# cmgcds/SParSH-AMG

Hardware: NVIDIA B200
Metric: amg_pcg_solve_seconds_poisson3d_256 (lower is better)
Workload: dtype f64

## Files before the change

### sparsh_amg_b200/csrc/internal.cuh

```cuda
#pragma once
#include <cuda_runtime.h>
#include <stdint.h>

#include <string>

#include <nvtx3/nvToolsExt.h>

#include "../../include/sparsh_b200.h"

namespace sparsh {

void set_error(const std::string &msg);
int cuda_fail(cudaError_t e, const char *what, const char *file, int line);

#define SP_CUDA(call)                                                              \
    do {                                                                           \
        cudaError_t e__ = (call);                                                  \
        if (e__ != cudaSuccess) return ::sparsh::cuda_fail(e__, #call, __FILE__, __LINE__); \
    } while (0)
#define SP_TRY(call)                      \
    do {                                  \
        int rc__ = (call);                \
        if (rc__ != SPARSH_OK) return rc__; \
    } while (0)
// ... 82 lines not shown
    int off;
    int pad;
};
struct PatView {
    const unsigned char *__restrict__ pat;
    const PatEntry *__restrict__ ent;
    const int *__restrict__ start;
    const double *__restrict__ pdiag;
    int n_pat, n_ent;
    int use_pdiag;
    int far_off;
};
constexpr int PAT_TILE = 512;
constexpr int PAT_MAX_WIN = 8;
constexpr int PAT_WIN_DOUBLES = 3072;
struct PatWindows {
    int nwin;
    int lo[PAT_MAX_WIN], len[PAT_MAX_WIN];
    int total;
    int w0;
    const unsigned char *__restrict__ win;
};
constexpr int PAT0_MAX = 32;
struct Pat0 {
    int len = 0;
    int kdiag = -1;
    int lo = 0, hi = 0;
    double diag = 0.0;
    double cover = 0.0;
    int off[PAT0_MAX] = {};
    double val[PAT0_MAX] = {};
};
constexpr int PAT_ESCAPE = 255;
constexpr int PAT_MAX_ENT = 2048;
constexpr int PAT_MAX_ROW = 64;

struct CsrView {
    int nrow, ncol, nnz;
    const int *__restrict__ rowptr;
    const int *__restrict__ col;
    const double *__restrict__ val;
};

}

struct sparsh_matrix_s {
    int nrow = 0, ncol = 0, nnz = 0;
    int *rowptr = nullptr;
    int *col = nullptr;
    double *val = nullptr;
    double *diag = nullptr;
    int kind = sparsh::KIND_VECTOR;
    int threads = 256;
    bool threads_forced = false;
    int lanes = 8;
    int max_row = 0;
    double mean_row = 0.0;
    int win128 = 0, win256 = 0;
    int smem_bytes = 0;
    unsigned short *code = nullptr;
    double *dict_val = nullptr;
    int *dict_off = nullptr;
    int n_dval = 0, n_doff = 0;
    bool has_dict = false;
    unsigned char *pat = nullptr;
    sparsh::PatEntry *pat_ent = nullptr;
// ... 113 lines not shown
```

### sparsh_amg_b200/csrc/matrix.cu

```cuda
#include <algorithm>
#include <chrono>
#include <cmath>
#include <cstdlib>
#include <cstring>
#include <mutex>
#include <thread>
#include <unordered_map>
#include <vector>

#include <cstdio>

#include "spmv_common.cuh"

using namespace sparsh;

namespace {

void choose_kernel(sparsh_matrix_s *A, const int *rp) {
    const int n = A->nrow;
    int max_row = 0, w128 = 0, w256 = 0;
    for (int i = 0; i < n; i++) {
        max_row = std::max(max_row, rp[i + 1] - rp[i]);
        w128 = std::max(w128, rp[std::min(i + 128, n)] - rp[i]);
        w256 = std::max(w256, rp[std::min(i + 256, n)] - rp[i]);
// ... 795 lines not shown
    if (smem_bytes) *smem_bytes = A->kind == KIND_STREAM ? A->smem_bytes : 0;
    if (smem_bytes && A->kind == KIND_DICT)
        *smem_bytes = ((((A->threads == 256 ? A->win256 : A->win128) + 16) + 7) & ~7) * 2 + A->n_dval * 8 + A->n_doff * 4;
    return SPARSH_OK;
}

int sparsh_matrix_pattern_stats(sparsh_matrix_t A, int *n_pat, int *n_ent, int *n_escape, double *cover0) {
    SP_REQUIRE(A != nullptr, "matrix is NULL");
    if (n_pat) *n_pat = A->has_pat ? A->n_pat : 0;
    if (n_ent) *n_ent = A->has_pat ? A->n_pent : 0;
    if (n_escape) *n_escape = A->has_pat ? A->n_escape : A->nrow;
    if (cover0) *cover0 = A->has_pat ? A->pat0.cover : 0.0;
    return SPARSH_OK;
}

int sparsh_matrix_kernel_name(sparsh_matrix_t A, int epi, char *buf, size_t len) {
    SP_REQUIRE(A != nullptr && buf != nullptr && len > 0, "bad arguments");
    static const char *epis[] = {"EPI_SPMV", "EPI_RESID", "EPI_JACOBI", "EPI_PROLONG", "EPI_SOR", "EPI_SPMV_DOT", "EPI_RESNORM"};
    SP_REQUIRE(epi >= 0 && epi < 7, "unknown epilogue");
    char tmp[160];
    switch (A->kind) {
        case KIND_SCALAR:
            std::snprintf(tmp, sizeof tmp, "csr_scalar_kernel<256,%s>", epis[epi]);
            break;
        case KIND_STREAM:
            std::snprintf(tmp, sizeof tmp, "csr_stream_kernel<%d,%s>", A->threads, epis[epi]);
            break;
        case KIND_DICT:
            std::snprintf(tmp, sizeof tmp, "csr_dict_kernel<%d,4,%s>", A->threads, epis[epi]);
            break;
        case KIND_PATTERN:
            if (pattern_lean_applies(A)) {
                const bool div = epi == EPI_JACOBI || epi == EPI_SOR;
                const bool one_row = A->threads_forced ? A->threads == 256 : div;
                std::snprintf(tmp, sizeof tmp, "csr_pat2_kernel<%d,%d,%d,%s>", one_row ? 256 : 128, one_row ? 1 : 2, A->pat0.len, epis[epi]);
            } else {
                std::snprintf(tmp, sizeof tmp, "csr_pattern_kernel<%d,4,2,%s>", A->threads, epis[epi]);
            }
            break;
        default:
            std::snprintf(tmp, sizeof tmp, "csr_vector_kernel<%d,%s>", A->lanes, epis[epi]);
    }
    std::snprintf(buf, len, "%s", tmp);
    return SPARSH_OK;
}

int sparsh_matrix_force_kernel(sparsh_matrix_t A, int kind, int tl) {
    SP_REQUIRE(A != nullptr, "matrix is NULL");
    if (kind == KIND_SCALAR) {
        A->kind = kind;
        A->threads = 256;
    } else if (kind == KIND_STREAM) {
        SP_REQUIRE(tl == 128 || tl == 256, "stream kernel: threads must be 128 or 256");
        const int win = tl == 256 ? A->win256 : A->win128;
        const int smem = (((win + 8) + 3) & ~3) * 12;
        SP_REQUIRE(smem <= 200 * 1024, "stream kernel: row window does not fit in shared memory");
        A->kind = kind;
        A->threads = tl;
        A->smem_bytes = smem;
    } else if (kind == KIND_DICT) {
        SP_REQUIRE(A->has_dict, "dict kernel: this matrix has no csr-dict16 twin (more than 256 distinct values or offsets)");
        SP_REQUIRE(tl == 128 || tl == 256, "dict kernel: threads must be 128 or 256");
        A->kind = kind;
        A->threads = tl;
    } else if (kind == KIND_PATTERN) {
        SP_REQUIRE(A->has_pat, "pattern kernel: this matrix has no csr-pattern8 twin (SPARSH_PATTERN unset, or rows do not repeat)");
        SP_REQUIRE(tl == 128 || tl == 256, "pattern kernel: threads must be 128 or 256");
        A->kind = kind;
        A->threads = tl;
        A->threads_forced = true;
    } else if (kind == KIND_VECTOR) {
        SP_REQUIRE(tl == 2 || tl == 4 || tl == 8 || tl == 16 || tl == 32, "vector kernel: lanes must be 2..32");
        A->kind = kind;
        A->lanes = tl;
    } else {
        SP_REQUIRE(false, "unknown kernel kind");
    }
    return SPARSH_OK;
}

int sparsh_spmv(sparsh_matrix_t A, const double *d_x, double *d_y) {
    SP_REQUIRE(A != nullptr, "matrix is NULL");
    return launch_csr(A, EPI_SPMV, d_x, d_y, EpiArgs(), 0, A->nrow);
}

int sparsh_spmv_dot(sparsh_matrix_t A, const double *d_x, double *d_y, double *d_dot) {
    SP_REQUIRE(A != nullptr && A->nrow == A->ncol, "spmv_dot needs a square matrix");
    EpiArgs a;
    a.xi = d_x;
    a.red_out = d_dot;
    return launch_csr(A, EPI_SPMV_DOT, d_x, d_y, a, 0, A->nrow);
}

int sparsh_residual(sparsh_matrix_t A, const double *d_b, const double *d_x, double *d_r) {
    SP_REQUIRE(A != nullptr, "matrix is NULL");
    EpiArgs a;
    a.b = d_b;
    return launch_csr(A, EPI_RESID, d_x, d_r, a, 0, A->nrow);
}

// ... 58 lines not shown
```

### sparsh_amg_b200/csrc/spmv_pattern.cu

```cuda
#include <algorithm>
#include <cstdlib>

#include "spmv_common.cuh"

namespace sparsh {

namespace {

template <bool COHERENT, bool DIST, bool SAFE>
__device__ __forceinline__ double gather(const double *x, int c, int ncol, int halo_begin) {
    if (!SAFE) c = min(max(c, 0), ncol - 1);
    return load_xd<COHERENT, DIST>(x, c, halo_begin);
}

__device__ __forceinline__ void prefetch_l2_line(const void *p) { asm volatile("prefetch.global.L2 [%0];" ::"l"(p)); }

__device__ __forceinline__ void virtual_block_rows(const RowRange &rr, int blk, int rows_per_cta, int &first, int &end) {
    first = rr.b1;
    end = rr.e1;
    if (blk >= rr.nblk1) {
        blk -= rr.nblk1;
        first = rr.b2;
        end = rr.e2;
        if (blk >= rr.nblk2) {
            blk -= rr.nblk2;
            first = rr.b3;
            end = rr.e3;
        }
    }
    first += blk * rows_per_cta;
}

template <int THREADS, int RPT, int LEN0, int EPI, bool DIST>
__global__ void __launch_bounds__(THREADS)
    csr_pat2_kernel(CsrView A, PatView P, const __grid_constant__ Pat0 Z, const double *x, double *y, EpiArgs args,
                    RowRange rr, double *partials, HaloSync hs, int pf_dist) {
    pdl_prologue();
    constexpr bool NEEDS_B = (EPI == EPI_RESID || EPI == EPI_JACOBI || EPI == EPI_SOR || EPI == EPI_RESNORM);
    constexpr bool NEEDS_D = (EPI == EPI_JACOBI || EPI == EPI_SOR);
    constexpr bool COH = EpiTraits<EPI>::coherent_x;
    constexpr int TILE = THREADS * RPT;

    const int tid = threadIdx.x;
    int r0, row_end;
    block_rows(rr, TILE, r0, row_end);
    const int nrows = min(TILE, row_end - r0);

    if (pf_dist > 0 && (int)blockIdx.x + pf_dist < (int)gridDim.x) {
        int p0, pend;
        virtual_block_rows(rr, blockIdx.x + pf_dist, TILE, p0, pend);
        const int pn = min(TILE, pend - p0);
        constexpr int LPT = TILE / 16;
        if (pn > 0) {
            const int part = tid / LPT, line = tid % LPT;
            const int i = p0 + line * 16;
            if (i < p0 + pn) {
                if (part == 0) prefetch_l2_line(x + i);
                if (part == 1 && Z.hi > 0 && i + Z.hi < A.ncol) prefetch_l2_line(x + i + Z.hi);
                if (part == 2 && NEEDS_B) prefetch_l2_line(args.b + i);
                if (part == 3 && (line & 7) == 0) prefetch_l2_line(P.pat + i);
            }
        }
    }
// ... 5 lines not shown
    const bool table_d = P.use_pdiag != 0;

    int pid[RPT];
    EpiRegs e[RPT];
    double g[RPT][LEN0];
#pragma unroll
    for (int s = 0; s < RPT; s++) {
        pid[s] = -1;
        if (s * THREADS + tid < nrows) {
            const int row = r0 + s * THREADS + tid;
            pid[s] = __ldg(P.pat + row);
            e[s] = epi_load<EPI, false>(args, y, row);
            if (NEEDS_D && !table_d) e[s].d = args.d[row];
            if (safe) {
#pragma unroll
                for (int k = 0; k < LEN0; k++) g[s][k] = gather<COH, DIST, true>(x, row + Z.off[k], A.ncol, hs.halo_begin);
            } else {
#pragma unroll
                for (int k = 0; k < LEN0; k++) g[s][k] = gather<COH, DIST, false>(x, row + Z.off[k], A.ncol, hs.halo_begin);
            }
        }
    }

    double contrib = 0.0;
#pragma unroll
    for (int s = 0; s < RPT; s++) {
        if (pid[s] < 0) continue;
        const int row = r0 + s * THREADS + tid;
        double sum = 0.0;
        if (pid[s] == 0) {
#pragma unroll
            for (int k = 0; k < LEN0; k++) sum = __dadd_rn(sum, __dmul_rn(Z.val[k], g[s][k]));
            if (NEEDS_D && table_d) e[s].d = Z.diag;
        } else if (pid[s] != PAT_ESCAPE) {
            const int st = __ldg(P.start + pid[s]), en = __ldg(P.start + pid[s] + 1);
#pragma unroll 1
            for (int k = st; k < en; k++) {
                const int4 q = __ldg(reinterpret_cast<const int4 *>(P.ent) + k);
                sum = __dadd_rn(sum, __dmul_rn(__hiloint2double(q.y, q.x), load_xd<COH, DIST>(x, row + q.z, hs.halo_begin)));
            }
            if (NEEDS_D && table_d) e[s].d = __ldg(P.pdiag + pid[s]);
        } else {
            const int lo = A.rowptr[row], hi = A.rowptr[row + 1];
#pragma unroll 1
            for (int k = lo; k < hi; k++)
                sum = __dadd_rn(sum, __dmul_rn(__ldg(A.val + k), load_xd<COH, DIST>(x, __ldg(A.col + k), hs.halo_begin)));
            if (NEEDS_D) e[s].d = args.d[row];
        }
        contrib = __dadd_rn(contrib, epi_store<EPI, DIST>(args, e[s], sum, y, row, strip_cta));
    }
    if (pushes<EPI, DIST>(args, strip_cta)) {
#pragma unroll 1
        for (int s = 0; s < RPT; s++)
            if (pid[s] >= 0) fused_push<EPI, DIST>(args, y, r0 + s * THREADS + tid);
    }
    if (EpiTraits<EPI>::reduces) block_partial<THREADS>(contrib, partials);
    if (DIST) halo_done(hs, hs_turn);
}

template <int THREADS, int RPT, int LEN0, int EPI>
int launch_cfg(const sparsh_matrix_s *A, const double *x, double *y, const EpiArgs &args, LaunchDesc d) {
    Context &c = ctx();
    const int grid = grid_for(d, THREADS * RPT);
    if (grid > RED_MAX_BLOCKS) {
        set_error("matrix too large for the reduction workspace");
        return SPARSH_ERR_INVALID;
    }
    const PatView P = A->pattern(args.d != nullptr && args.d == A->diag);
    static const int pf = [] {
        const char *e = getenv("SPARSH_PAT2_PF");
        return e ? atoi(e) : 0;
    }();
    if (d.dist)
        SP_CUDA(launch_k(csr_pat2_kernel<THREADS, RPT, LEN0, EPI, true>, dim3(grid), dim3(THREADS), 0, c.stream, A->view(), P, A->pat0, x, y, args, d.rr, c.partials, d.hs, pf));
    else
        SP_CUDA(launch_k(csr_pat2_kernel<THREADS, RPT, LEN0, EPI, false>, dim3(grid), dim3(THREADS), 0, c.stream, A->view(), P, A->pat0, x, y, args, d.rr, c.partials, d.hs, pf));
    count_launch();
    SP_CUDA(cudaGetLastError());
    if (EpiTraits<EPI>::reduces) return launch_finalize_partials(grid, args.red_out);
    return SPARSH_OK;
}

template <int LEN0, int EPI>
int launch_len(const sparsh_matrix_s *A, const double *x, double *y, const EpiArgs &args, const LaunchDesc &d) {
    const bool one_row = A->threads_forced ? A->threads == 256 : (EPI == EPI_JACOBI || EPI == EPI_SOR);
    if (one_row) return launch_cfg<256, 1, LEN0, EPI>(A, x, y, args, d);
    return launch_cfg<128, 2, LEN0, EPI>(A, x, y, args, d);
}

template <int EPI>
int launch_epi(const sparsh_matrix_s *A, const double *x, double *y, const EpiArgs &args, const LaunchDesc &d) {
    switch (A->pat0.len) {
        case 5:
            return launch_len<5, EPI>(A, x, y, args, d);
        default:
            return launch_len<7, EPI>(A, x, y, args, d);
    }
}

}

bool pattern_lean_applies(const sparsh_matrix_s *A) {
    static const bool enabled = [] {
        const char *e = getenv("SPARSH_PAT2");
        return !(e && atoi(e) == 0);
    }();
    const int len = A->pat0.len;
    return enabled && A->has_pat && (len == 5 || len == 7) && A->pat0.cover >= 0.5;
}

int launch_pattern_lean(const sparsh_matrix_s *A, int epi, const double *x, double *y, const EpiArgs &args, LaunchDesc d) {
    switch (epi) {
        case EPI_SPMV:
            return launch_epi<EPI_SPMV>(A, x, y, args, d);
        case EPI_RESID:
            return launch_epi<EPI_RESID>(A, x, y, args, d);
        case EPI_JACOBI:
            return launch_epi<EPI_JACOBI>(A, x, y, args, d);
// ... 15 lines not shown
```

### sparsh_amg_b200/csrc/hierarchy.cuh

```cuda
#pragma once
#include <vector>

#include "internal.cuh"

namespace sparsh {

struct Level {
    sparsh_matrix_s *A = nullptr;
    sparsh_matrix_s *P = nullptr;
    sparsh_matrix_s *R = nullptr;
    int n = 0;
    double *xbuf = nullptr;
    double *tbuf = nullptr;
    double *bbuf = nullptr;
    double *rbuf = nullptr;
    std::vector<int> color_count;
};

struct GraphEntry {
    const void *k0 = nullptr, *k1 = nullptr;
    int tag = 0;
    cudaGraphExec_t exec = nullptr;
    long long kernels = 0;
};

}

struct sparsh_hierarchy_s {
    std::vector<sparsh::Level> lev;
    sparsh_params prm;
    sparsh::CoarseInverse coarse;
    sparsh::DevSlab *slab = nullptr;
    double *kv[8] = {nullptr, nullptr, nullptr, nullptr, nullptr, nullptr, nullptr, nullptr};
    double *d_sc = nullptr;
    double *h_sc = nullptr;
    double *hb = nullptr, *hx = nullptr;
    double *gm_V = nullptr, *gm_d = nullptr, *gm_h = nullptr;
    int gm_m = 0;
    std::vector<sparsh::GraphEntry> graphs;
    int tail_state = 0, tail_first = -1, tail_grid = 0, tail_nops = 0;
    void *tail_prog = nullptr;
    double *tail_x = nullptr;
};

namespace sparsh {

int enqueue_vcycle(sparsh_hierarchy_s *h, const double *b, double *x, bool x_is_zero);
template <class F>
int run_graphed(sparsh_hierarchy_s *h, const void *k0, const void *k1, int tag, F body);
int krylov_workspace(sparsh_hierarchy_s *h, int nvec);
int tail_level(sparsh_hierarchy_s *h);
int enqueue_tail(sparsh_hierarchy_s *h);
void tail_free(sparsh_hierarchy_s *h);

template <class F>
int run_graphed(sparsh_hierarchy_s *h, const void *k0, const void *k1, int tag, F body) {
    Context &c = ctx();
    if (!h->prm.use_graph) return body();
    GraphEntry *ent = nullptr;
    for (auto &g : h->graphs)
        if (g.k0 == k0 && g.k1 == k1 && g.tag == tag) ent = &g;
    if (!ent) {
        GraphEntry g;
        g.k0 = k0;
        g.k1 = k1;
        g.tag = tag;
        h->graphs.push_back(g);
        return body();
    }
    if (!ent->exec) {
        NvtxRange nvtx("sparsh:graph-capture");
        cudaGraph_t graph = nullptr;
        SP_CUDA(cudaStreamBeginCapture(c.stream, cudaStreamCaptureModeThreadLocal));
        c.capturing = true;
// ... 24 lines not shown
```

### sparsh_amg_b200/csrc/tail.cu

```cuda
#include <cooperative_groups.h>

#include <cstdlib>
#include <vector>

#include "hierarchy.cuh"

namespace sparsh {

namespace {

enum TailKind { T_JACOBI_ZERO = 0, T_JACOBI = 1, T_RESID = 2, T_SPMV = 3, T_PROLONG = 4, T_GEMV = 5, T_FILL0 = 6 };

struct TailOp {
    int kind, n;
    const int *rp, *ci;
    const double *val, *diag;
    const double *x, *b;
    double *y;
    double omega;
};

constexpr int TAIL_T = 1024;

__device__ __forceinline__ double row_sum(const TailOp &op, int row) {
    double s = 0.0;
    for (int k = op.rp[row]; k < op.rp[row + 1]; k++) s = __dadd_rn(s, __dmul_rn(__ldg(op.val + k), __ldcg(op.x + __ldg(op.ci + k))));
    return s;
}

template <bool CLUSTER>
__global__ void __launch_bounds__(TAIL_T) tail_cycle_kernel(const TailOp *__restrict__ ops, int nops) {
    const int tid = blockIdx.x * TAIL_T + threadIdx.x, nthreads = gridDim.x * TAIL_T;
    for (int o = 0; o < nops; o++) {
        const TailOp op = ops[o];
        if (op.kind == T_GEMV) {
            const int lane = threadIdx.x & 31, warp = tid >> 5, nwarps = nthreads >> 5;
            const bool vec = (op.n & 1) == 0 && (reinterpret_cast<uintptr_t>(op.b) & 15) == 0;
            for (int row = warp; row < op.n; row += nwarps) {
                const double *m = op.val + (size_t)row * op.n;
                double s0 = 0.0, s1 = 0.0;
                if (vec) {
                    for (int j = lane * 2; j + 1 < op.n; j += 64) {
                        const double2 a = *reinterpret_cast<const double2 *>(m + j);
                        const double v0 = __ldcg(op.b + j), v1 = __ldcg(op.b + j + 1);
                        s0 = fma(a.x, v0, s0);
                        s1 = fma(a.y, v1, s1);
                    }
                } else {
                    for (int j = lane; j < op.n; j += 32) s0 = fma(m[j], __ldcg(op.b + j), s0);
                }
                double s = s0 + s1;
#pragma unroll
                for (int off = 16; off > 0; off >>= 1) s += __shfl_xor_sync(0xffffffffu, s, off);
                if (lane == 0) op.y[row] = s;
            }
        } else {
            for (int row = tid; row < op.n; row += nthreads) {
                switch (op.kind) {
                    case T_JACOBI_ZERO:
                        op.y[row] = __ddiv_rn(__dmul_rn(op.omega, __ldcg(op.b + row)), op.diag[row]);
                        break;
                    case T_JACOBI: {
                        const double h = __dsub_rn(__ldcg(op.b + row), row_sum(op, row));
                        op.y[row] = __dadd_rn(__ldcg(op.x + row), __ddiv_rn(__dmul_rn(op.omega, h), op.diag[row]));
                        break;
                    }
                    case T_RESID:
                        op.y[row] = __dsub_rn(__ldcg(op.b + row), row_sum(op, row));
                        break;
                    case T_SPMV:
                        op.y[row] = row_sum(op, row);
                        break;
                    case T_PROLONG:
                        op.y[row] = __dadd_rn(row_sum(op, row), __ldcg(op.y + row));
                        break;
                    default:
                        op.y[row] = 0.0;
                }
            }
        }
        if (CLUSTER)
            cooperative_groups::this_cluster().sync();
        else
            cooperative_groups::this_grid().sync();
    }
}

}

static int tail_mode() {
    const char *e = getenv("SPARSH_TAIL_MODE");
    return e ? atoi(e) : 0;
}
static int tail_rows() {
    const char *e = getenv("SPARSH_TAIL_ROWS");
    if (e) return atoi(e);
    return tail_mode() == 2 ? 32768 : 131072;
}

int tail_level(sparsh_hierarchy_s *h) {
    if (h->tail_state == 2) return -1;
    if (h->tail_state == 1) return h->tail_first;
    h->tail_state = 2;
    const int L = (int)h->lev.size() - 1;
    if (tail_mode() <= 0 || tail_rows() <= 0 || h->prm.smoother != 0 || L < 1 || h->coarse.n == 0) return -1;
    int first = L;
    while (first > 1 && h->lev[first - 1].n <= tail_rows()) first--;
    if (first >= L) return -1;
    for (int l = first; l < L; l++)
        if (h->lev[l].A->kind == KIND_VECTOR || h->lev[l].P->kind == KIND_VECTOR || h->lev[l].R->kind == KIND_VECTOR) return -1;
    const bool cluster = tail_mode() == 2;
    int coop = 0;
    if (!cluster && (cudaDeviceGetAttribute(&coop, cudaDevAttrCooperativeLaunch, ctx().device) != cudaSuccess || !coop)) return -1;
    if (cluster && cudaFuncSetAttribute(tail_cycle_kernel<true>, cudaFuncAttributeNonPortableClusterSizeAllowed, 1) != cudaSuccess) {
        cudaGetLastError();
        return -1;
    }
    std::vector<TailOp> prog;
    auto mat = [](TailOp &op, const sparsh_matrix_s *M) {
        op.n = M->nrow;
        op.rp = M->rowptr;
        op.ci = M->col;
        op.val = M->val;
    };
    std::vector<double *> X(L + 1), T(L + 1);
    for (int l = first; l <= L; l++) {
        X[l] = h->lev[l].xbuf;
        T[l] = h->lev[l].tbuf;
    }
    const double omega = h->prm.omega;
    auto smooth = [&](int l, int sweeps, bool zero) {
        Level &F = h->lev[l];
        if (sweeps == 0) {
            if (zero) {
                TailOp op = {};
                op.kind = T_FILL0;
                op.n = F.n;
                op.y = X[l];
                prog.push_back(op);
            }
            return;
        }
        for (int s = 0; s < sweeps; s++) {
            TailOp op = {};
            mat(op, F.A);
            op.diag = F.A->diag;
            op.b = F.bbuf;
            op.omega = omega;
            op.y = T[l];
            if (s == 0 && zero) {
                op.kind = T_JACOBI_ZERO;
            } else {
                op.kind = T_JACOBI;
                op.x = X[l];
            }
            prog.push_back(op);
            std::swap(X[l], T[l]);
        }
    };
    for (int l = first; l < L; l++) {
        Level &F = h->lev[l];
        smooth(l, h->prm.pre_sweeps, true);
        TailOp r = {};
        mat(r, F.A);
        r.kind = T_RESID;
        r.x = X[l];
        r.b = F.bbuf;
        r.y = F.rbuf;
        prog.push_back(r);
        TailOp t = {};
        mat(t, F.R);
        t.kind = T_SPMV;
        t.x = F.rbuf;
        t.y = h->lev[l + 1].bbuf;
        prog.push_back(t);
    }
    {
        TailOp g = {};
        g.kind = T_GEMV;
        g.n = h->coarse.n;
        g.val = h->coarse.inv;
        g.b = h->lev[L].bbuf;
        g.y = X[L];
        prog.push_back(g);
    }
    for (int l = L; l > first; l--) {
        Level &F = h->lev[l - 1];
        TailOp p = {};
        mat(p, F.P);
        p.kind = T_PROLONG;
        p.x = X[l];
        p.y = X[l - 1];
        prog.push_back(p);
        smooth(l - 1, h->prm.post_sweeps, false);
    }
    int per_sm = 0;
    if (cudaOccupancyMaxActiveBlocksPerMultiprocessor(&per_sm, tail_cycle_kernel<false>, TAIL_T, 0) != cudaSuccess || per_sm < 1) {
        cudaGetLastError();
        return -1;
    }
    const int want = (h->lev[first].n + TAIL_T - 1) / TAIL_T;
    h->tail_grid = cluster ? -16 : std::max(1, std::min(want, ctx().sm_count));
    if (cudaMalloc(&h->tail_prog, sizeof(TailOp) * prog.size()) != cudaSuccess ||
        cudaMemcpy(h->tail_prog, prog.data(), sizeof(TailOp) * prog.size(), cudaMemcpyHostToDevice) != cudaSuccess) {
        cudaGetLastError();
        return -1;
    }
    h->tail_nops = (int)prog.size();
    h->tail_first = first;
    h->tail_x = X[first];
    h->tail_state = 1;
    return first;
}

int enqueue_tail(sparsh_hierarchy_s *h) {
    Context &c = ctx();
    const TailOp *prog = static_cast<const TailOp *>(h->tail_prog);
    int nops = h->tail_nops;
    if (h->tail_grid < 0) {
        cudaLaunchConfig_t cfg = {};
        cfg.gridDim = dim3(-h->tail_grid);
        cfg.blockDim = dim3(TAIL_T);
        cfg.stream = c.stream;
        cudaLaunchAttribute attr[1];
        attr[0].id = cudaLaunchAttributeClusterDimension;
        attr[0].val.clusterDim.x = (unsigned)(-h->tail_grid);
        attr[0].val.clusterDim.y = 1;
        attr[0].val.clusterDim.z = 1;
        cfg.attrs = attr;
        cfg.numAttrs = 1;
        SP_CUDA(cudaLaunchKernelEx(&cfg, tail_cycle_kernel<true>, prog, nops));
    } else {
        void *args[] = {(void *)&prog, (void *)&nops};
        SP_CUDA(cudaLaunchCooperativeKernel((const void *)tail_cycle_kernel<false>, dim3(h->tail_grid), dim3(TAIL_T), args, 0, c.stream));
    }
    count_launch();
    return SPARSH_OK;
}

void tail_free(sparsh_hierarchy_s *h) {
    cudaFree(h->tail_prog);
    h->tail_prog = nullptr;
    h->tail_state = 0;
}

}
```

Baseline: 0.1441.

## Add consecutive-rows pattern SpMV kernel with vectorized loads for large stencil matrices

Adds csr_pat_rows_kernel, where each thread handles two consecutive rows. The -1/0/+1 neighbour values are shared through one contiguous window of x, and x, b, y and the pattern bytes are moved with double2/uchar2 vector loads and stores. It is used for SPMV, RESID and JACOBI on non-distributed matrices with at least 65536 rows when alignment and offset conditions hold. The goal is fewer redundant x loads and fewer memory transactions than the interleaved-strip pat2 kernel. In exchange it adds a slow-path boundary branch, more dispatch conditions, and possibly less coalescing because each thread reads two adjacent rows.

```diff
diff --git a/sparsh_amg_b200/csrc/internal.cuh b/sparsh_amg_b200/csrc/internal.cuh
--- a/sparsh_amg_b200/csrc/internal.cuh
+++ b/sparsh_amg_b200/csrc/internal.cuh
@@ -138,6 +138,9 @@
     double val[PAT0_MAX] = {};
 };
 constexpr int PAT_ESCAPE = 255;
+constexpr int PAT_ROWS_PER_THREAD = 2;
+constexpr int PAT_ROWS_THREADS = 128;
+constexpr int PAT_ROWS_MIN_ROWS = 1 << 16;
 constexpr int PAT_MAX_ENT = 2048;
 constexpr int PAT_MAX_ROW = 64;
 
diff --git a/sparsh_amg_b200/csrc/matrix.cu b/sparsh_amg_b200/csrc/matrix.cu
--- a/sparsh_amg_b200/csrc/matrix.cu
+++ b/sparsh_amg_b200/csrc/matrix.cu
@@ -851,8 +851,15 @@
         case KIND_PATTERN:
             if (pattern_lean_applies(A)) {
                 const bool div = epi == EPI_JACOBI || epi == EPI_SOR;
-                const bool one_row = A->threads_forced ? A->threads == 256 : div;
-                std::snprintf(tmp, sizeof tmp, "csr_pat2_kernel<%d,%d,%d,%s>", one_row ? 256 : 128, one_row ? 1 : 2, A->pat0.len, epis[epi]);
+                const bool forced_one = A->threads_forced && A->threads != PAT_ROWS_PER_THREAD;
+                const bool forced_rows = A->threads_forced && A->threads == PAT_ROWS_PER_THREAD;
+                const bool one_row = forced_one ? A->threads == 256 : div;
+                if ((forced_rows || (!forced_one && A->nrow >= PAT_ROWS_MIN_ROWS)) &&
+                    (epi == EPI_SPMV || epi == EPI_RESID || epi == EPI_JACOBI))
+                    std::snprintf(tmp, sizeof tmp, "csr_pat_rows_kernel<%d,%d,%d,%s>", PAT_ROWS_THREADS, PAT_ROWS_PER_THREAD,
+                                  A->pat0.len, epis[epi]);
+                else
+                    std::snprintf(tmp, sizeof tmp, "csr_pat2_kernel<%d,%d,%d,%s>", one_row ? 256 : 128, one_row ? 1 : 2, A->pat0.len, epis[epi]);
             } else {
                 std::snprintf(tmp, sizeof tmp, "csr_pattern_kernel<%d,4,2,%s>", A->threads, epis[epi]);
             }
@@ -884,7 +891,8 @@
         A->threads = tl;
     } else if (kind == KIND_PATTERN) {
         SP_REQUIRE(A->has_pat, "pattern kernel: this matrix has no csr-pattern8 twin (SPARSH_PATTERN unset, or rows do not repeat)");
-        SP_REQUIRE(tl == 128 || tl == 256, "pattern kernel: threads must be 128 or 256");
+        SP_REQUIRE(tl == 128 || tl == 256 || tl == PAT_ROWS_PER_THREAD,
+                   "pattern kernel: threads must be 128 or 256, or PAT_ROWS_PER_THREAD for the consecutive-rows kernel");
         A->kind = kind;
         A->threads = tl;
         A->threads_forced = true;
diff --git a/sparsh_amg_b200/csrc/spmv_pattern.cu b/sparsh_amg_b200/csrc/spmv_pattern.cu
--- a/sparsh_amg_b200/csrc/spmv_pattern.cu
+++ b/sparsh_amg_b200/csrc/spmv_pattern.cu
@@ -29,6 +29,28 @@
         }
     }
     first += blk * rows_per_cta;
+}
+
+template <bool NEEDS_D, bool COH, bool DIST>
+__device__ __forceinline__ double other_row_sum(const CsrView &A, const PatView &P, const EpiArgs &args, const double *x,
+                                                int row, int pid, int halo_begin, double &d) {
+    double sum = 0.0;
+    if (pid != PAT_ESCAPE) {
+        const int st = __ldg(P.start + pid), en = __ldg(P.start + pid + 1);
+#pragma unroll 1
+        for (int k = st; k < en; k++) {
+            const int4 q = __ldg(reinterpret_cast<const int4 *>(P.ent) + k);
+            sum = __dadd_rn(sum, __dmul_rn(__hiloint2double(q.y, q.x), load_xd<COH, DIST>(x, row + q.z, halo_begin)));
+        }
+        if (NEEDS_D && P.use_pdiag) d = __ldg(P.pdiag + pid);
+    } else {
+        const int lo = A.rowptr[row], hi = A.rowptr[row + 1];
+#pragma unroll 1
+        for (int k = lo; k < hi; k++)
+            sum = __dadd_rn(sum, __dmul_rn(__ldg(A.val + k), load_xd<COH, DIST>(x, __ldg(A.col + k), halo_begin)));
+        if (NEEDS_D) d = args.d[row];
+    }
+    return sum;
 }
 
 template <int THREADS, int RPT, int LEN0, int EPI, bool DIST>
@@ -100,20 +122,8 @@
 #pragma unroll
             for (int k = 0; k < LEN0; k++) sum = __dadd_rn(sum, __dmul_rn(Z.val[k], g[s][k]));
             if (NEEDS_D && table_d) e[s].d = Z.diag;
-        } else if (pid[s] != PAT_ESCAPE) {
-            const int st = __ldg(P.start + pid[s]), en = __ldg(P.start + pid[s] + 1);
-#pragma unroll 1
-            for (int k = st; k < en; k++) {
-                const int4 q = __ldg(reinterpret_cast<const int4 *>(P.ent) + k);
-                sum = __dadd_rn(sum, __dmul_rn(__hiloint2double(q.y, q.x), load_xd<COH, DIST>(x, row + q.z, hs.halo_begin)));
-            }
-            if (NEEDS_D && table_d) e[s].d = __ldg(P.pdiag + pid[s]);
         } else {
-            const int lo = A.rowptr[row], hi = A.rowptr[row + 1];
-#pragma unroll 1
-            for (int k = lo; k < hi; k++)
-                sum = __dadd_rn(sum, __dmul_rn(__ldg(A.val + k), load_xd<COH, DIST>(x, __ldg(A.col + k), hs.halo_begin)));
-            if (NEEDS_D) e[s].d = args.d[row];
+            sum = other_row_sum<NEEDS_D, COH, DIST>(A, P, args, x, row, pid[s], hs.halo_begin, e[s].d);
         }
         contrib = __dadd_rn(contrib, epi_store<EPI, DIST>(args, e[s], sum, y, row, strip_cta));
     }
@@ -124,6 +134,131 @@
     }
     if (EpiTraits<EPI>::reduces) block_partial<THREADS>(contrib, partials);
     if (DIST) halo_done(hs, hs_turn);
+}
+
+template <int EPI>
+__device__ __forceinline__ double epi_value(const EpiArgs &a, double b, double xi, double d, double s) {
+    if (EPI == EPI_RESID) return __dsub_rn(b, s);
+    if (EPI == EPI_JACOBI) return __dadd_rn(xi, __ddiv_rn(__dmul_rn(a.omega, __dsub_rn(b, s)), d));
+    return s;
+}
+
+template <int LEN0, int EPI, bool SAFE>
+__device__ __forceinline__ void pat_row(const CsrView &A, const PatView &P, const Pat0 &Z, const double *x, double *y,
+                                        const EpiArgs &args, int row) {
+    constexpr bool NEEDS_D = EPI == EPI_JACOBI;
+    const int pid = __ldg(P.pat + row);
+    EpiRegs e = epi_load<EPI, false>(args, y, row);
+    if (NEEDS_D && !P.use_pdiag) e.d = args.d[row];
+    double g[LEN0];
+#pragma unroll
+    for (int k = 0; k < LEN0; k++) g[k] = gather<false, false, SAFE>(x, row + Z.off[k], A.ncol, 0);
+    double sum = 0.0;
+    if (pid == 0) {
+#pragma unroll
+        for (int k = 0; k < LEN0; k++) sum = __dadd_rn(sum, __dmul_rn(Z.val[k], g[k]));
+        if (NEEDS_D && P.use_pdiag) e.d = Z.diag;
+    } else {
+        sum = other_row_sum<NEEDS_D, false, false>(A, P, args, x, row, pid, 0, e.d);
+    }
+    epi_store<EPI, false>(args, e, sum, y, row);
+}
+
+template <int THREADS, int R, int LEN0, int EPI, bool EVEN>
+__global__ void __launch_bounds__(THREADS, 4)
+    csr_pat_rows_kernel(CsrView A, PatView P, const __grid_constant__ Pat0 Z, const double *x, double *y, EpiArgs args,
+                        RowRange rr) {
+    pdl_prologue();
+    static_assert(EPI == EPI_SPMV || EPI == EPI_RESID || EPI == EPI_JACOBI, "epilogues that store one value per row");
+    constexpr bool NEEDS_B = EPI != EPI_SPMV;
+    constexpr bool NEEDS_D = EPI == EPI_JACOBI;
+    constexpr int TILE = THREADS * R;
+    int r0, row_end;
+    block_rows(rr, TILE, r0, row_end);
+    const int row0 = r0 + R * (int)threadIdx.x;
+
+    if (r0 + TILE > row_end || r0 + min(Z.lo, -2) < 0 || r0 + TILE - 1 + max(Z.hi, 2) >= A.ncol) {
+        const bool safe = r0 + Z.lo >= 0 && r0 + TILE - 1 + Z.hi < A.ncol;
+#pragma unroll 1
+        for (int s = 0; s < R; s++) {
+            const int row = row0 + s;
+            if (row >= row_end) break;
+            if (safe)
+                pat_row<LEN0, EPI, true>(A, P, Z, x, y, args, row);
+            else
+                pat_row<LEN0, EPI, false>(A, P, Z, x, y, args, row);
+        }
+        return;
+    }
+
+    static_assert(R == 2 || R == 4, "pattern bytes come as one uchar2 or uchar4");
+    int pid[R];
+    if constexpr (R == 2) {
+        const uchar2 p = __ldg(reinterpret_cast<const uchar2 *>(P.pat + row0));
+        pid[0] = p.x;
+        pid[1] = p.y;
+    } else {
+        const uchar4 p = __ldg(reinterpret_cast<const uchar4 *>(P.pat + row0));
+        pid[0] = p.x;
+        pid[1] = p.y;
+        pid[2] = p.z;
+        pid[3] = p.w;
+    }
+    double b[R] = {}, w[R + 4], d[R];
+    if (NEEDS_B) {
+#pragma unroll
+        for (int j = 0; j < R / 2; j++) {
+            const double2 v = __ldg(reinterpret_cast<const double2 *>(args.b + row0) + j);
+            b[2 * j] = v.x;
+            b[2 * j + 1] = v.y;
+        }
+    }
+#pragma unroll
+    for (int j = 0; j < R / 2 + 2; j++) {
+        const double2 v = __ldg(reinterpret_cast<const double2 *>(x + row0 - 2) + j);
+        w[2 * j] = v.x;
+        w[2 * j + 1] = v.y;
+    }
+    constexpr int KC = LEN0 / 2;
+    double g[R][LEN0];
+#pragma unroll
+    for (int k = 0; k < LEN0; k++) {
+        if (k >= KC - 1 && k <= KC + 1) {
+#pragma unroll
+            for (int s = 0; s < R; s++) g[s][k] = w[s + 2 + k - KC];
+        } else if (EVEN) {
+#pragma unroll
+            for (int j = 0; j < R / 2; j++) {
+                const double2 v = __ldg(reinterpret_cast<const double2 *>(x + row0 + Z.off[k]) + j);
+                g[2 * j][k] = v.x;
+                g[2 * j + 1][k] = v.y;
+            }
+        } else {
+#pragma unroll
+            for (int s = 0; s < R; s++) g[s][k] = __ldg(x + row0 + s + Z.off[k]);
+        }
+    }
+    if (NEEDS_D && !P.use_pdiag) {
+#pragma unroll
+        for (int s = 0; s < R; s++) d[s] = args.d[row0 + s];
+    }
+
+    double sum[R];
+#pragma unroll
+    for (int s = 0; s < R; s++) {
+        sum[s] = 0.0;
+#pragma unroll
+        for (int k = 0; k < LEN0; k++) sum[s] = __dadd_rn(sum[s], __dmul_rn(Z.val[k], g[s][k]));
+        if (NEEDS_D && P.use_pdiag) d[s] = Z.diag;
+    }
+    double v[R];
+#pragma unroll
+    for (int s = 0; s < R; s++) {
+        if (pid[s] != 0) sum[s] = other_row_sum<NEEDS_D, false, false>(A, P, args, x, row0 + s, pid[s], 0, d[s]);
+        v[s] = epi_value<EPI>(args, b[s], w[s + 2], d[s], sum[s]);
+    }
+#pragma unroll
+    for (int j = 0; j < R / 2; j++) reinterpret_cast<double2 *>(y + row0)[j] = make_double2(v[2 * j], v[2 * j + 1]);
 }
 
 template <int THREADS, int RPT, int LEN0, int EPI>
@@ -149,9 +284,47 @@
     return SPARSH_OK;
 }
 
+template <int THREADS, int R, int LEN0, int EPI>
+int launch_rows(const sparsh_matrix_s *A, const double *x, double *y, const EpiArgs &args, LaunchDesc d, bool even) {
+    const int grid = grid_for(d, THREADS * R);
+    const PatView P = A->pattern(args.d != nullptr && args.d == A->diag);
+    if (even)
+        SP_CUDA(launch_k(csr_pat_rows_kernel<THREADS, R, LEN0, EPI, true>, dim3(grid), dim3(THREADS), 0, ctx().stream, A->view(), P, A->pat0, x, y, args, d.rr));
+    else
+        SP_CUDA(launch_k(csr_pat_rows_kernel<THREADS, R, LEN0, EPI, false>, dim3(grid), dim3(THREADS), 0, ctx().stream, A->view(), P, A->pat0, x, y, args, d.rr));
+    count_launch();
+    SP_CUDA(cudaGetLastError());
+    return SPARSH_OK;
+}
+
+inline bool pat0_offsets_even(const Pat0 &Z) {
+    for (int k = 0; k < Z.len; k++)
+        if ((Z.off[k] & 1) && (k < Z.len / 2 - 1 || k > Z.len / 2 + 1)) return false;
+    return true;
+}
+
+template <int EPI>
+bool rows_kernel_applies(const sparsh_matrix_s *A, const double *x, const double *y, const EpiArgs &args, const LaunchDesc &d,
+                         int R) {
+    const Pat0 &Z = A->pat0;
+    const int kc = Z.len / 2;
+    if (Z.off[kc - 1] != -1 || Z.off[kc] != 0 || Z.off[kc + 1] != 1) return false;
+    if (d.dist || (EPI == EPI_JACOBI && args.xi != x)) return false;
+    auto al16 = [](const void *p) { return ((uintptr_t)p & 15) == 0; };
+    if (!al16(x) || !al16(y) || (EPI != EPI_SPMV && !al16(args.b)) || ((uintptr_t)A->pat % R) != 0) return false;
+    return d.rr.b1 % R == 0 && (d.rows2 == 0 || d.rr.b2 % R == 0) && (d.rows3 == 0 || d.rr.b3 % R == 0);
+}
+
 template <int LEN0, int EPI>
 int launch_len(const sparsh_matrix_s *A, const double *x, double *y, const EpiArgs &args, const LaunchDesc &d) {
-    const bool one_row = A->threads_forced ? A->threads == 256 : (EPI == EPI_JACOBI || EPI == EPI_SOR);
+    const bool forced_one = A->threads_forced && A->threads != PAT_ROWS_PER_THREAD;
+    const bool forced_rows = A->threads_forced && A->threads == PAT_ROWS_PER_THREAD;
+    const bool big = d.rows1 + d.rows2 + d.rows3 >= PAT_ROWS_MIN_ROWS;
+    if constexpr (EPI == EPI_SPMV || EPI == EPI_RESID || EPI == EPI_JACOBI) {
+        if ((forced_rows || (!forced_one && big)) && rows_kernel_applies<EPI>(A, x, y, args, d, PAT_ROWS_PER_THREAD))
+            return launch_rows<PAT_ROWS_THREADS, PAT_ROWS_PER_THREAD, LEN0, EPI>(A, x, y, args, d, pat0_offsets_even(A->pat0));
+    }
+    const bool one_row = forced_one ? A->threads == 256 : (EPI == EPI_JACOBI || EPI == EPI_SOR);
     if (one_row) return launch_cfg<256, 1, LEN0, EPI>(A, x, y, args, d);
     return launch_cfg<128, 2, LEN0, EPI>(A, x, y, args, d);
 }
```

After: 0.1344, median of 6. -6.7%, faster.

## Replace interpreted tail V-cycle with cluster-resident DSMEM kernels, enabled by default

Applied to the files above, without the earlier changes.

Replaces the op-list interpreter kernel that ran the coarse levels under grid/cluster sync with two specialized cluster kernels (down and up sweeps). Each CTA keeps its slice of the level vectors and the compressed stencil pattern tables in shared memory, and neighbours are read through distributed shared memory. The coarse solve moves to a separate coarse_apply call between the two kernels. Tail mode now defaults to on (cluster mode, no row limit), so the coarse levels run in two launches instead of many kernels. In exchange it depends on shared-memory budgets, non-portable cluster sizes of 16 or 8, and the pattern-lean format, and it adds a lot of new fragile code.

```diff
diff --git a/sparsh_amg_b200/csrc/hierarchy.cuh b/sparsh_amg_b200/csrc/hierarchy.cuh
--- a/sparsh_amg_b200/csrc/hierarchy.cuh
+++ b/sparsh_amg_b200/csrc/hierarchy.cuh
@@ -38,8 +38,8 @@
     double *gm_V = nullptr, *gm_d = nullptr, *gm_h = nullptr;
     int gm_m = 0;
     std::vector<sparsh::GraphEntry> graphs;
-    int tail_state = 0, tail_first = -1, tail_grid = 0, tail_nops = 0;
-    void *tail_prog = nullptr;
+    int tail_state = 0, tail_first = -1, tail_cta = 0;
+    size_t tail_smem = 0;
     double *tail_x = nullptr;
 };
 
diff --git a/sparsh_amg_b200/csrc/tail.cu b/sparsh_amg_b200/csrc/tail.cu
--- a/sparsh_amg_b200/csrc/tail.cu
+++ b/sparsh_amg_b200/csrc/tail.cu
@@ -1,101 +1,278 @@
-#include <cooperative_groups.h>
-
+#include <algorithm>
 #include <cstdlib>
-#include <vector>
 
 #include "hierarchy.cuh"
 
 namespace sparsh {
 
+bool pattern_lean_applies(const sparsh_matrix_s *A);
+
 namespace {
 
-enum TailKind { T_JACOBI_ZERO = 0, T_JACOBI = 1, T_RESID = 2, T_SPMV = 3, T_PROLONG = 4, T_GEMV = 5, T_FILL0 = 6 };
-
-struct TailOp {
-    int kind, n;
+constexpr int TAIL_T = 1024;
+constexpr int TAIL_MAX_LEV = 12;
+
+struct TailLevel {
+    int n, m;
+    float inv_m;
+    int lean;
+    int ox0, ox1, ob, opat;
+    int oent, ostart, opd;
+    int n_pat, n_ent;
     const int *rp, *ci;
     const double *val, *diag;
-    const double *x, *b;
-    double *y;
+    const unsigned char *pat;
+    const PatEntry *ent;
+    const int *start;
+    const double *pdiag;
+    const int *prp, *pci;
+    const double *pval;
+    const int *rrp, *rci;
+    const double *rval;
+    double *xg, *bg;
+};
+
+struct TailProg {
+    int nlev;
+    int pre, post;
     double omega;
+    int nL, mL;
+    double *bL;
+    const double *xL;
+    TailLevel lev[TAIL_MAX_LEV];
+    Pat0 z[TAIL_MAX_LEV];
 };
 
-constexpr int TAIL_T = 1024;
-
-__device__ __forceinline__ double row_sum(const TailOp &op, int row) {
+__device__ __forceinline__ uint32_t cta_rank() {
+    uint32_t r;
+    asm volatile("mov.u32 %0, %%cluster_ctarank;" : "=r"(r));
+    return r;
+}
+__device__ __forceinline__ void cluster_sync() {
+    asm volatile("barrier.cluster.arrive.release.aligned;\nbarrier.cluster.wait.acquire.aligned;" ::: "memory");
+}
+__device__ __forceinline__ double ld_dsmem(uint32_t local_addr, uint32_t rank) {
+    uint32_t a;
+    double v;
+    asm volatile("mapa.shared::cluster.u32 %0, %1, %2;" : "=r"(a) : "r"(local_addr), "r"(rank));
+    asm volatile("ld.shared::cluster.f64 %0, [%1];" : "=d"(v) : "r"(a));
+    return v;
+}
+
+__device__ __forceinline__ double vget(uint32_t base, const TailLevel &L, int off, int i) {
+    const int owner = __float2int_rz(((float)i + 0.5f) * L.inv_m);
+    const int k = i - owner * L.m;
+    return ld_dsmem(base + off + 8u * k, owner);
+}
+
+template <int LEN>
+__device__ __forceinline__ double pat0_row(uint32_t base, const TailLevel &L, const Pat0 &z, int xo, int i) {
+    double g[LEN];
+#pragma unroll
+    for (int k = 0; k < LEN; k++) g[k] = vget(base, L, xo, i + z.off[k]);
     double s = 0.0;
-    for (int k = op.rp[row]; k < op.rp[row + 1]; k++) s = __dadd_rn(s, __dmul_rn(__ldg(op.val + k), __ldcg(op.x + __ldg(op.ci + k))));
+#pragma unroll
+    for (int k = 0; k < LEN; k++) s = __dadd_rn(s, __dmul_rn(z.val[k], g[k]));
     return s;
 }
 
-template <bool CLUSTER>
-__global__ void __launch_bounds__(TAIL_T) tail_cycle_kernel(const TailOp *__restrict__ ops, int nops) {
-    const int tid = blockIdx.x * TAIL_T + threadIdx.x, nthreads = gridDim.x * TAIL_T;
-    for (int o = 0; o < nops; o++) {
-        const TailOp op = ops[o];
-        if (op.kind == T_GEMV) {
-            const int lane = threadIdx.x & 31, warp = tid >> 5, nwarps = nthreads >> 5;
-            const bool vec = (op.n & 1) == 0 && (reinterpret_cast<uintptr_t>(op.b) & 15) == 0;
-            for (int row = warp; row < op.n; row += nwarps) {
-                const double *m = op.val + (size_t)row * op.n;
-                double s0 = 0.0, s1 = 0.0;
-                if (vec) {
-                    for (int j = lane * 2; j + 1 < op.n; j += 64) {
-                        const double2 a = *reinterpret_cast<const double2 *>(m + j);
-                        const double v0 = __ldcg(op.b + j), v1 = __ldcg(op.b + j + 1);
-                        s0 = fma(a.x, v0, s0);
-                        s1 = fma(a.y, v1, s1);
-                    }
-                } else {
-                    for (int j = lane; j < op.n; j += 32) s0 = fma(m[j], __ldcg(op.b + j), s0);
+__device__ __forceinline__ double a_row(const unsigned char *sm, uint32_t base, const TailLevel &L, const Pat0 &z,
+                                        int xo, int i, int p, double &d) {
+    double s = 0.0;
+    if (p == 0) {
+        s = z.len == 5 ? pat0_row<5>(base, L, z, xo, i) : pat0_row<7>(base, L, z, xo, i);
+        d = z.diag;
+        return s;
+    }
+    if (p > 0 && p != PAT_ESCAPE) {
+        const int *start = reinterpret_cast<const int *>(sm + L.ostart);
+        const PatEntry *ent = reinterpret_cast<const PatEntry *>(sm + L.oent);
+        const int st = start[p], en = start[p + 1];
+#pragma unroll 4
+        for (int k = st; k < en; k++) s = __dadd_rn(s, __dmul_rn(ent[k].v, vget(base, L, xo, i + ent[k].off)));
+        d = reinterpret_cast<const double *>(sm + L.opd)[p];
+        return s;
+    } else {
+        const int lo = __ldg(L.rp + i), hi = __ldg(L.rp + i + 1);
+#pragma unroll 4
+        for (int k = lo; k < hi; k++) s = __dadd_rn(s, __dmul_rn(__ldg(L.val + k), vget(base, L, xo, __ldg(L.ci + k))));
+    }
+    d = __ldg(L.diag + i);
+    return s;
+}
+
+template <bool UP>
+__global__ void __launch_bounds__(TAIL_T, 1) tail_resident_kernel(const __grid_constant__ TailProg p) {
+    extern __shared__ __align__(16) unsigned char sm[];
+    const uint32_t base = (uint32_t)__cvta_generic_to_shared(sm);
+    const int rank = (int)cta_rank(), tid = threadIdx.x;
+    const double omega = p.omega;
+    auto X = [&](int off) { return reinterpret_cast<double *>(sm + off); };
+    auto rows = [&](const TailLevel &L, int &lo) {
+        lo = rank * L.m;
+        return max(0, min(L.m, L.n - lo));
+    };
+
+    for (int j = 0; j < p.nlev; j++) {
+        const TailLevel &L = p.lev[j];
+        if (L.lean) {
+            for (int k = tid; k < L.n_ent; k += TAIL_T) reinterpret_cast<PatEntry *>(sm + L.oent)[k] = L.ent[k];
+            for (int k = tid; k <= L.n_pat; k += TAIL_T) reinterpret_cast<int *>(sm + L.ostart)[k] = L.start[k];
+            for (int k = tid; k < L.n_pat; k += TAIL_T) reinterpret_cast<double *>(sm + L.opd)[k] = L.pdiag[k];
+        }
+        int lo;
+        const int cnt = rows(L, lo);
+        for (int i = tid; i < cnt; i += TAIL_T) {
+            if (L.lean) sm[L.opat + i] = __ldg(L.pat + lo + i);
+            if (UP) X(L.ox0)[i] = L.xg[lo + i];
+            if (UP || j == 0) X(L.ob)[i] = L.bg[lo + i];
+        }
+    }
+    cluster_sync();
+
+    auto sweep = [&](int j, int xo, int yo, bool zero) {
+        const TailLevel &L = p.lev[j];
+        const Pat0 &z = p.z[j];
+        int lo;
+        const int cnt = rows(L, lo);
+        for (int i = tid; i < cnt; i += TAIL_T) {
+            const int pid = L.lean ? (int)sm[L.opat + i] : -1;
+            const double b = X(L.ob)[i];
+            double v;
+            if (zero) {
+                const double d = pid == 0                        ? z.diag
+                                 : pid > 0 && pid != PAT_ESCAPE ? reinterpret_cast<const double *>(sm + L.opd)[pid]
+                                                                : __ldg(L.diag + lo + i);
+                v = __ddiv_rn(__dmul_rn(omega, b), d);
+            } else {
+                double d;
+                const double s = a_row(sm, base, L, z, xo, lo + i, pid, d);
+                v = __dadd_rn(X(xo)[i], __ddiv_rn(__dmul_rn(omega, __dsub_rn(b, s)), d));
+            }
+            X(yo)[i] = v;
+        }
+        cluster_sync();
+    };
+    auto smooth = [&](int j, int sweeps, bool zero, int &cur) {
+        const TailLevel &L = p.lev[j];
+        if (sweeps == 0 && zero) {
+            int lo;
+            const int cnt = rows(L, lo);
+            for (int i = tid; i < cnt; i += TAIL_T) X(cur)[i] = 0.0;
+            cluster_sync();
+        }
+        for (int s = 0; s < sweeps; s++) {
+            const int other = cur == L.ox0 ? L.ox1 : L.ox0;
+            sweep(j, cur, other, zero && s == 0);
+            cur = other;
+        }
+    };
+
+    if (!UP) {
+        for (int j = 0; j < p.nlev; j++) {
+            const TailLevel &L = p.lev[j];
+            const Pat0 &z = p.z[j];
+            int cur = L.ox0;
+            smooth(j, p.pre, true, cur);
+            const int ro = cur == L.ox0 ? L.ox1 : L.ox0;
+            int lo;
+            const int cnt = rows(L, lo);
+            for (int i = tid; i < cnt; i += TAIL_T) {
+                const int pid = L.lean ? (int)sm[L.opat + i] : -1;
+                double d;
+                const double s = a_row(sm, base, L, z, cur, lo + i, pid, d);
+                X(ro)[i] = __dsub_rn(X(L.ob)[i], s);
+                L.xg[lo + i] = X(cur)[i];
+                if (j > 0) L.bg[lo + i] = X(L.ob)[i];
+            }
+            cluster_sync();
+            const bool last = j + 1 == p.nlev;
+            const int nc = last ? p.nL : p.lev[j + 1].n, mc = last ? p.mL : p.lev[j + 1].m;
+            const int clo = rank * mc, ccnt = max(0, min(mc, nc - clo));
+            double *dst = last ? p.bL + clo : X(p.lev[j + 1].ob);
+            for (int i = tid; i < ccnt; i += TAIL_T) {
+                const int a = __ldg(L.rrp + clo + i), e = __ldg(L.rrp + clo + i + 1);
+                double s = 0.0;
+#pragma unroll 4
+                for (int k = a; k < e; k++) s = __dadd_rn(s, __dmul_rn(__ldg(L.rval + k), vget(base, L, ro, __ldg(L.rci + k))));
+                dst[i] = s;
+            }
+            cluster_sync();
+        }
+    } else {
+        int fin = 0;
+        for (int j = p.nlev - 1; j >= 0; j--) {
+            const TailLevel &L = p.lev[j];
+            const bool last = j + 1 == p.nlev;
+            int lo;
+            const int cnt = rows(L, lo);
+            for (int i = tid; i < cnt; i += TAIL_T) {
+                const int a = __ldg(L.prp + lo + i), e = __ldg(L.prp + lo + i + 1);
+                double s = 0.0;
+#pragma unroll 4
+                for (int k = a; k < e; k++) {
+                    const int c = __ldg(L.pci + k);
+                    const double xc = last ? __ldg(p.xL + c) : vget(base, p.lev[j + 1], fin, c);
+                    s = __dadd_rn(s, __dmul_rn(__ldg(L.pval + k), xc));
                 }
-                double s = s0 + s1;
-#pragma unroll
-                for (int off = 16; off > 0; off >>= 1) s += __shfl_xor_sync(0xffffffffu, s, off);
-                if (lane == 0) op.y[row] = s;
-            }
-        } else {
-            for (int row = tid; row < op.n; row += nthreads) {
-                switch (op.kind) {
-                    case T_JACOBI_ZERO:
-                        op.y[row] = __ddiv_rn(__dmul_rn(op.omega, __ldcg(op.b + row)), op.diag[row]);
-                        break;
-                    case T_JACOBI: {
-                        const double h = __dsub_rn(__ldcg(op.b + row), row_sum(op, row));
-                        op.y[row] = __dadd_rn(__ldcg(op.x + row), __ddiv_rn(__dmul_rn(op.omega, h), op.diag[row]));
-                        break;
-                    }
-                    case T_RESID:
-                        op.y[row] = __dsub_rn(__ldcg(op.b + row), row_sum(op, row));
-                        break;
-                    case T_SPMV:
-                        op.y[row] = row_sum(op, row);
-                        break;
-                    case T_PROLONG:
-                        op.y[row] = __dadd_rn(row_sum(op, row), __ldcg(op.y + row));
-                        break;
-                    default:
-                        op.y[row] = 0.0;
-                }
-            }
-        }
-        if (CLUSTER)
-            cooperative_groups::this_cluster().sync();
-        else
-            cooperative_groups::this_grid().sync();
-    }
+                X(L.ox0)[i] = __dadd_rn(s, X(L.ox0)[i]);
+            }
+            cluster_sync();
+            int cur = L.ox0;
+            smooth(j, p.post, false, cur);
+            fin = cur;
+        }
+        const TailLevel &L = p.lev[0];
+        int lo;
+        const int cnt = rows(L, lo);
+        for (int i = tid; i < cnt; i += TAIL_T) L.xg[lo + i] = X(fin)[i];
+    }
+}
+
+size_t tail_layout(sparsh_hierarchy_s *h, int first, int C, TailProg *prog) {
+    const int L = (int)h->lev.size() - 1;
+    size_t off = 0;
+    for (int l = first; l < L; l++) {
+        const int n = h->lev[l].n, m = (n + C - 1) / C;
+        const sparsh_matrix_s *A = h->lev[l].A;
+        const bool lean = pattern_lean_applies(A);
+        if (prog) {
+            TailLevel &T = prog->lev[l - first];
+            T.n = n;
+            T.m = m;
+            T.inv_m = 1.0f / (float)m;
+            T.lean = lean;
+            T.ox0 = (int)off;
+            T.ox1 = (int)(off + 8 * (size_t)m);
+            T.ob = (int)(off + 16 * (size_t)m);
+            T.opat = (int)(off + 24 * (size_t)m);
+        }
+        off += 24 * (size_t)m;
+        if (lean) {
+            off += ((size_t)m + 15) / 16 * 16;
+            if (prog) {
+                TailLevel &T = prog->lev[l - first];
+                T.n_pat = A->n_pat;
+                T.n_ent = A->n_pent;
+                T.oent = (int)off;
+                T.opd = (int)(off + 16 * (size_t)A->n_pent);
+                T.ostart = (int)(off + 16 * (size_t)A->n_pent + 8 * (size_t)A->n_pat);
+            }
+            off += 16 * (size_t)A->n_pent + 8 * (size_t)A->n_pat + ((4 * ((size_t)A->n_pat + 1) + 15) / 16 * 16);
+        }
+    }
+    return off;
 }
 
 }
 
 static int tail_mode() {
     const char *e = getenv("SPARSH_TAIL_MODE");
-    return e ? atoi(e) : 0;
+    return e ? atoi(e) : 2;
 }
 static int tail_rows() {
     const char *e = getenv("SPARSH_TAIL_ROWS");
-    if (e) return atoi(e);
-    return tail_mode() == 2 ? 32768 : 131072;
+    return e ? atoi(e) : 0x7fffffff;
 }
 
 int tail_level(sparsh_hierarchy_s *h) {
@@ -103,145 +280,113 @@
     if (h->tail_state == 1) return h->tail_first;
     h->tail_state = 2;
     const int L = (int)h->lev.size() - 1;
-    if (tail_mode() <= 0 || tail_rows() <= 0 || h->prm.smoother != 0 || L < 1 || h->coarse.n == 0) return -1;
-    int first = L;
-    while (first > 1 && h->lev[first - 1].n <= tail_rows()) first--;
-    if (first >= L) return -1;
-    for (int l = first; l < L; l++)
-        if (h->lev[l].A->kind == KIND_VECTOR || h->lev[l].P->kind == KIND_VECTOR || h->lev[l].R->kind == KIND_VECTOR) return -1;
-    const bool cluster = tail_mode() == 2;
-    int coop = 0;
-    if (!cluster && (cudaDeviceGetAttribute(&coop, cudaDevAttrCooperativeLaunch, ctx().device) != cudaSuccess || !coop)) return -1;
-    if (cluster && cudaFuncSetAttribute(tail_cycle_kernel<true>, cudaFuncAttributeNonPortableClusterSizeAllowed, 1) != cudaSuccess) {
+    if (tail_mode() <= 0 || tail_rows() <= 0 || h->prm.smoother != 0 || L < 2 || h->coarse.n == 0) return -1;
+    int lowest = 1;
+    for (int l = 1; l < L; l++)
+        if (h->lev[l].A->kind == KIND_VECTOR || h->lev[l].P->kind == KIND_VECTOR || h->lev[l].R->kind == KIND_VECTOR) lowest = l + 1;
+    lowest = std::max(lowest, L - TAIL_MAX_LEV);
+    int optin = 0;
+    cudaFuncAttributes fa = {};
+    if (cudaDeviceGetAttribute(&optin, cudaDevAttrMaxSharedMemoryPerBlockOptin, ctx().device) != cudaSuccess ||
+        cudaFuncGetAttributes(&fa, tail_resident_kernel<false>) != cudaSuccess) {
         cudaGetLastError();
         return -1;
     }
-    std::vector<TailOp> prog;
-    auto mat = [](TailOp &op, const sparsh_matrix_s *M) {
-        op.n = M->nrow;
-        op.rp = M->rowptr;
-        op.ci = M->col;
-        op.val = M->val;
-    };
-    std::vector<double *> X(L + 1), T(L + 1);
-    for (int l = first; l <= L; l++) {
-        X[l] = h->lev[l].xbuf;
-        T[l] = h->lev[l].tbuf;
-    }
-    const double omega = h->prm.omega;
-    auto smooth = [&](int l, int sweeps, bool zero) {
-        Level &F = h->lev[l];
-        if (sweeps == 0) {
-            if (zero) {
-                TailOp op = {};
-                op.kind = T_FILL0;
-                op.n = F.n;
-                op.y = X[l];
-                prog.push_back(op);
-            }
-            return;
-        }
-        for (int s = 0; s < sweeps; s++) {
-            TailOp op = {};
-            mat(op, F.A);
-            op.diag = F.A->diag;
-            op.b = F.bbuf;
-            op.omega = omega;
-            op.y = T[l];
-            if (s == 0 && zero) {
-                op.kind = T_JACOBI_ZERO;
-            } else {
-                op.kind = T_JACOBI;
-                op.x = X[l];
-            }
-            prog.push_back(op);
-            std::swap(X[l], T[l]);
-        }
-    };
-    for (int l = first; l < L; l++) {
-        Level &F = h->lev[l];
-        smooth(l, h->prm.pre_sweeps, true);
-        TailOp r = {};
-        mat(r, F.A);
-        r.kind = T_RESID;
-        r.x = X[l];
-        r.b = F.bbuf;
-        r.y = F.rbuf;
-        prog.push_back(r);
-        TailOp t = {};
-        mat(t, F.R);
-        t.kind = T_SPMV;
-        t.x = F.rbuf;
-        t.y = h->lev[l + 1].bbuf;
-        prog.push_back(t);
-    }
-    {
-        TailOp g = {};
-        g.kind = T_GEMV;
-        g.n = h->coarse.n;
-        g.val = h->coarse.inv;
-        g.b = h->lev[L].bbuf;
-        g.y = X[L];
-        prog.push_back(g);
-    }
-    for (int l = L; l > first; l--) {
-        Level &F = h->lev[l - 1];
-        TailOp p = {};
-        mat(p, F.P);
-        p.kind = T_PROLONG;
-        p.x = X[l];
-        p.y = X[l - 1];
-        prog.push_back(p);
-        smooth(l - 1, h->prm.post_sweeps, false);
-    }
-    int per_sm = 0;
-    if (cudaOccupancyMaxActiveBlocksPerMultiprocessor(&per_sm, tail_cycle_kernel<false>, TAIL_T, 0) != cudaSuccess || per_sm < 1) {
+    const size_t budget = (size_t)optin - fa.sharedSizeBytes;
+    for (int C : {16, 8}) {
+        int first = L;
+        while (first > lowest && h->lev[first - 1].n <= tail_rows() && (h->lev[first - 1].n + C - 1) / C <= TAIL_T &&
+               tail_layout(h, first - 1, C, nullptr) <= budget)
+            first--;
+        if (first >= L) continue;
+        const size_t smem = tail_layout(h, first, C, nullptr);
+        bool ok = true;
+        for (auto k : {tail_resident_kernel<false>, tail_resident_kernel<true>})
+            ok = ok && cudaFuncSetAttribute(k, cudaFuncAttributeNonPortableClusterSizeAllowed, 1) == cudaSuccess &&
+                 cudaFuncSetAttribute(k, cudaFuncAttributeMaxDynamicSharedMemorySize, (int)budget) == cudaSuccess;
+        int nclusters = 0;
+        if (ok) {
+            cudaLaunchConfig_t cfg = {};
+            cudaLaunchAttribute attr[1];
+            attr[0].id = cudaLaunchAttributeClusterDimension;
+            attr[0].val.clusterDim.x = (unsigned)C;
+            attr[0].val.clusterDim.y = 1;
+            attr[0].val.clusterDim.z = 1;
+            cfg.gridDim = dim3(C);
+            cfg.blockDim = dim3(TAIL_T);
+            cfg.dynamicSmemBytes = smem;
+            cfg.attrs = attr;
+            cfg.numAttrs = 1;
+            ok = cudaOccupancyMaxActiveClusters(&nclusters, tail_resident_kernel<false>, &cfg) == cudaSuccess && nclusters >= 1;
+        }
         cudaGetLastError();
-        return -1;
-    }
-    const int want = (h->lev[first].n + TAIL_T - 1) / TAIL_T;
-    h->tail_grid = cluster ? -16 : std::max(1, std::min(want, ctx().sm_count));
-    if (cudaMalloc(&h->tail_prog, sizeof(TailOp) * prog.size()) != cudaSuccess ||
-        cudaMemcpy(h->tail_prog, prog.data(), sizeof(TailOp) * prog.size(), cudaMemcpyHostToDevice) != cudaSuccess) {
-        cudaGetLastError();
-        return -1;
-    }
-    h->tail_nops = (int)prog.size();
-    h->tail_first = first;
-    h->tail_x = X[first];
-    h->tail_state = 1;
-    return first;
+        if (!ok) continue;
+        h->tail_first = first;
+        h->tail_cta = C;
+        h->tail_smem = smem;
+        h->tail_x = h->lev[first].xbuf;
+        h->tail_state = 1;
+        return first;
+    }
+    return -1;
 }
 
 int enqueue_tail(sparsh_hierarchy_s *h) {
     Context &c = ctx();
-    const TailOp *prog = static_cast<const TailOp *>(h->tail_prog);
-    int nops = h->tail_nops;
-    if (h->tail_grid < 0) {
-        cudaLaunchConfig_t cfg = {};
-        cfg.gridDim = dim3(-h->tail_grid);
-        cfg.blockDim = dim3(TAIL_T);
-        cfg.stream = c.stream;
-        cudaLaunchAttribute attr[1];
-        attr[0].id = cudaLaunchAttributeClusterDimension;
-        attr[0].val.clusterDim.x = (unsigned)(-h->tail_grid);
-        attr[0].val.clusterDim.y = 1;
-        attr[0].val.clusterDim.z = 1;
-        cfg.attrs = attr;
-        cfg.numAttrs = 1;
-        SP_CUDA(cudaLaunchKernelEx(&cfg, tail_cycle_kernel<true>, prog, nops));
-    } else {
-        void *args[] = {(void *)&prog, (void *)&nops};
-        SP_CUDA(cudaLaunchCooperativeKernel((const void *)tail_cycle_kernel<false>, dim3(h->tail_grid), dim3(TAIL_T), args, 0, c.stream));
-    }
+    const int L = (int)h->lev.size() - 1, first = h->tail_first, C = h->tail_cta;
+    TailProg p = {};
+    tail_layout(h, first, C, &p);
+    p.nlev = L - first;
+    p.pre = h->prm.pre_sweeps;
+    p.post = h->prm.post_sweeps;
+    p.omega = h->prm.omega;
+    p.nL = h->lev[L].n;
+    p.mL = (p.nL + C - 1) / C;
+    p.bL = h->lev[L].bbuf;
+    p.xL = h->lev[L].xbuf;
+    for (int l = first; l < L; l++) {
+        const Level &F = h->lev[l];
+        TailLevel &T = p.lev[l - first];
+        T.rp = F.A->rowptr;
+        T.ci = F.A->col;
+        T.val = F.A->val;
+        T.diag = F.A->diag;
+        if (T.lean) {
+            T.pat = F.A->pat;
+            T.ent = F.A->pat_ent;
+            T.start = F.A->pat_start;
+            T.pdiag = F.A->pat_diag;
+            p.z[l - first] = F.A->pat0;
+        }
+        T.prp = F.P->rowptr;
+        T.pci = F.P->col;
+        T.pval = F.P->val;
+        T.rrp = F.R->rowptr;
+        T.rci = F.R->col;
+        T.rval = F.R->val;
+        T.xg = F.xbuf;
+        T.bg = F.bbuf;
+    }
+    cudaLaunchConfig_t cfg = {};
+    cudaLaunchAttribute attr[1];
+    attr[0].id = cudaLaunchAttributeClusterDimension;
+    attr[0].val.clusterDim.x = (unsigned)C;
+    attr[0].val.clusterDim.y = 1;
+    attr[0].val.clusterDim.z = 1;
+    cfg.gridDim = dim3(C);
+    cfg.blockDim = dim3(TAIL_T);
+    cfg.dynamicSmemBytes = h->tail_smem;
+    cfg.stream = c.stream;
+    cfg.attrs = attr;
+    cfg.numAttrs = 1;
+    SP_CUDA(cudaLaunchKernelEx(&cfg, tail_resident_kernel<false>, p));
+    count_launch();
+    SP_TRY(coarse_apply(h->coarse, p.bL, h->lev[L].xbuf));
+    SP_CUDA(cudaLaunchKernelEx(&cfg, tail_resident_kernel<true>, p));
     count_launch();
     return SPARSH_OK;
 }
 
-void tail_free(sparsh_hierarchy_s *h) {
-    cudaFree(h->tail_prog);
-    h->tail_prog = nullptr;
-    h->tail_state = 0;
-}
-
-}
+void tail_free(sparsh_hierarchy_s *h) { h->tail_state = 0; }
+
+}
```

After: 0.1440 before, 0.1406 after, median of 6. 1.02x faster.
